# rpacheco-blazquez/PINN-FEM

Measured on AMD Instinct MI355X. Metric: element-residual-grad evals/sec (PINN+GD iteration: MLP fwd+bwd, stiffness, assembly, residual, Adam), collinear truss, higher is better.
Workload: dtype f32; 1 GPU; ex4 shape (nets (20, 15, 10), E and A evaluated), 1000000 elements per GPU, collinear 2-D truss h=1, alpha_data=100 with measurements at every node, load factor 0.1; elements_total=1000000, parallelism=elements sharded x1

## Files before the change

### include/pinnfem_hip.h

```cpp
#ifndef PINNFEM_HIP_H
#define PINNFEM_HIP_H

#include <stdint.h>

#ifdef __cplusplus
extern "C" {
#endif

#define PF_ABI_VERSION 8

#define PF_OK 0
#define PF_ERR_ARG (-1)
#define PF_ERR_UNSUPPORTED (-2)
#define PF_ERR_HIP (-3)

#define PF_DOF_FIXED 1u
#define PF_DOF_MEASURED 2u
#define PF_DOF_SHARED 4u
#define PF_DOF_GHOST 8u

#define PF_WG_SHUFFLE 0
#define PF_WG_MFMA 1
#define PF_WG_MFMA44 2
#define PF_WG_MFMA32 3
// ... 61 lines not shown
  int32_t wg_mode;
  float lam;
  float alpha_physics, alpha_data;
  float lr_u, lr_t;
  double tol;
  double beta1, beta2, eps;
  int32_t use_data;
  int32_t max_iter;
  float* theta_pad;
  float* prop_e;
  float* prop_a;
  float* g_f;
  float* g_ea;
  float* grad_u;
  float* grad_theta;
  float* partials;
  float* hist;
  pf_state* state;
  int32_t n_part_blocks;
  int32_t pad_total;
  const int32_t* pad_index;
  float n_meas_f;
  int32_t fe_mode;
  const int32_t* shared_dofs;
  const int32_t* shared_slot;
  int32_t n_shared;
  int32_t n_iface;
  int32_t own_lo, own_hi;
  int32_t part_half;
  int32_t prop_double;
  float* net_op;
  int32_t op_off[2];
  int32_t coord_exp;
  int32_t mlp_dtype;
  float* elem_k;
  float* theta_alt;
  float* u_alt;
  const int32_t* adj_other;
} pf_problem;

#define PF_MAX_BLOCKS 1024
#define PF_MAX_NODE_BLOCKS 4096
#define PF_NODE_SLOTS (PF_MAX_NODE_BLOCKS + 8)

int pf_abi_version(void);
const char* pf_last_error(void);
int pf_net_param_count(int in_dim, int width, int n_hidden);
int pf_padded_width(int width);
int pf_net_pad_count(int in_dim, int width, int n_hidden);
int pf_net_pad_index(int in_dim, int width, int n_hidden, int local);
int pf_sizeof(int what);
int pf_net_op_count(int in_dim, int width, int n_hidden);
long long pf_partials_count(const pf_problem* p);
#define PF_FUSED_FORWARD 1
#define PF_FUSED_BACKWARD 2
#define PF_FUSED_THETA_UPDATE 4
#define PF_FUSED_U_PINGPONG 8
#define PF_FUSED_U_UPDATE 16
int pf_fusion_info(const pf_problem* p);

int pf_pack_theta(const pf_problem* p, void* stream);
int pf_net_forward(const pf_problem* p, int which, void* stream);
int pf_net_forward_all(const pf_problem* p, void* stream);
int pf_net_backward_all(const pf_problem* p, void* stream);
int pf_internal_force(const pf_problem* p, const float* u, float* f_int_out, void* stream);
int pf_node_residual(const pf_problem* p, float* f_int_out, void* stream);
int pf_elem_adjoint(const pf_problem* p, void* stream);
int pf_net_backward(const pf_problem* p, int which, void* stream);
int pf_node_gradu(const pf_problem* p, int fuse_adam, void* stream);
int pf_theta_reduce(const pf_problem* p, int fuse_adam, void* stream);
int pf_finalize(const pf_problem* p, void* stream);
int pf_reset(const pf_problem* p, void* stream);

int pf_gd_iterations(const pf_problem* p, int n_iter, void* stream);
int pf_graph_create(const pf_problem* p, int iters_per_graph, void* stream, void** graph_out);
#define PF_GRAPH_CONT_HEAD 1
#define PF_GRAPH_NO_TAIL 2
int pf_graph_create_ex(const pf_problem* p, int iters_per_graph, int flags, void* stream, void** graph_out);
int pf_graph_tail(const pf_problem* p, int iters_per_graph, void* stream);
int pf_graph_launch(void* graph, void* stream);
int pf_graph_destroy(void* graph);
#define PF_KERNEL_SLOTS 9
int pf_gd_iterations_timed(const pf_problem* p, int n_iter, void* stream, float* ms_per_kernel);
int pf_loss_and_grads(const pf_problem* p, void* stream);

int pf_shard_forward(const pf_problem* p, void* stream);
int pf_shard_backward(const pf_problem* p, float* buf, const float* u2_local, void* stream);
int pf_shard_update_interior(const pf_problem* p, void* stream);
int pf_shard_update_shared(const pf_problem* p, const float* buf, float* u2_local, void* stream);
int pf_shard_flush(const pf_problem* p, const float* u2_reduced, void* stream);

#define PF_COMM_ID_BYTES 128
int pf_comm_unique_id(const char* librccl_path, void* id_out);
int pf_comm_create(const char* librccl_path, const void* id, int rank, int world, void** comm_out);
int pf_comm_destroy(void* comm);
int pf_comm_abort(void* comm);
int pf_comm_info(void* comm, int* rank_out, int* nranks_out);
int pf_comm_all_reduce(void* comm, float* buf, int n, void* stream);
int pf_shard_iterations(const pf_problem* p, void* comm, int n_iter, float* buf, float* u2_local, void* stream);
int pf_shard_graph_create(const pf_problem* p, void* comm, int iters_per_graph, float* buf, float* u2_local, void* stream,
                          void** graph_out);
int pf_shard_iterations_graph(const pf_problem* p, void* comm, void* graph, int iters_per_graph, int n_iter, float* buf,
                              float* u2_local, void* stream);

int pf_kv_f64(const pf_problem* p, const double* v, double* out, int zero_fixed, void* stream);
long long pf_pcg_workspace_count(const pf_problem* p);
// ... 53 lines not shown
```

### pinn_fem_amd/_capi.py

```python
from __future__ import annotations

import ctypes as C
import os

_HERE = os.path.dirname(os.path.abspath(__file__))
LIB_PATH = os.environ.get("PINNFEM_LIB") or os.path.join(_HERE, "lib", "libpinnfem_hip.so")

PF_ABI_VERSION = 8
PF_OK, PF_ERR_ARG, PF_ERR_UNSUPPORTED, PF_ERR_HIP = 0, -1, -2, -3
PF_DOF_FIXED, PF_DOF_MEASURED, PF_DOF_SHARED, PF_DOF_GHOST = 1, 2, 4, 8
PF_WG_SHUFFLE, PF_WG_MFMA, PF_WG_MFMA44, PF_WG_MFMA32 = 0, 1, 2, 3
PF_N32_WIDTH_MAX = 30
PF_MLP_F32, PF_MLP_BF16 = 0, 1
PF_FE_REFERENCE, PF_FE_DELTA = 0, 1
PF_HIST_COLS = 6
PF_MAX_BLOCKS = 1024
PF_COMM_ID_BYTES = 128
PF_MAX_NODE_BLOCKS = 4096
PF_NODE_SLOTS = PF_MAX_NODE_BLOCKS + 8
PF_KERNEL_SLOTS = 9
PF_COARSE_MAX_AGG, PF_COARSE_MODES = 256, 3
PF_COARSE_MAX = PF_COARSE_MAX_AGG * PF_COARSE_MODES
PF_GRAPH_CONT_HEAD, PF_GRAPH_NO_TAIL = 1, 2
PF_FUSED_FORWARD, PF_FUSED_BACKWARD, PF_FUSED_THETA_UPDATE, PF_FUSED_U_PINGPONG, PF_FUSED_U_UPDATE = 1, 2, 4, 8, 16
# ... 40 lines not shown
        ("theta", C.c_void_p), ("m_t", C.c_void_p), ("v_t", C.c_void_p),
        ("n_theta", C.c_int32), ("n_theta_active", C.c_int32),
        ("tensor_off", C.c_void_p),
        ("n_tensors", C.c_int32), ("wg_mode", C.c_int32),
        ("lam", C.c_float), ("alpha_physics", C.c_float), ("alpha_data", C.c_float),
        ("lr_u", C.c_float), ("lr_t", C.c_float),
        ("tol", C.c_double), ("beta1", C.c_double), ("beta2", C.c_double), ("eps", C.c_double),
        ("use_data", C.c_int32), ("max_iter", C.c_int32),
        ("theta_pad", C.c_void_p), ("prop_e", C.c_void_p), ("prop_a", C.c_void_p),
        ("g_f", C.c_void_p), ("g_ea", C.c_void_p), ("grad_u", C.c_void_p),
        ("grad_theta", C.c_void_p), ("partials", C.c_void_p), ("hist", C.c_void_p),
        ("state", C.c_void_p),
        ("n_part_blocks", C.c_int32), ("pad_total", C.c_int32),
        ("pad_index", C.c_void_p),
        ("n_meas_f", C.c_float), ("fe_mode", C.c_int32),
        ("shared_dofs", C.c_void_p), ("shared_slot", C.c_void_p),
        ("n_shared", C.c_int32), ("n_iface", C.c_int32),
        ("own_lo", C.c_int32), ("own_hi", C.c_int32), ("part_half", C.c_int32), ("prop_double", C.c_int32),
        ("net_op", C.c_void_p), ("op_off", C.c_int32 * 2), ("coord_exp", C.c_int32), ("mlp_dtype", C.c_int32),
        ("elem_k", C.c_void_p), ("theta_alt", C.c_void_p), ("u_alt", C.c_void_p), ("adj_other", C.c_void_p),
    ]


class PfScalarId(C.Structure):
    _fields_ = [
        ("p", C.c_void_p), ("m_p", C.c_void_p), ("v_p", C.c_void_p), ("table", C.c_void_p),
        ("n_rows", C.c_int32), ("has_bounds", C.c_int32),
        ("lo", C.c_float * 2), ("hi", C.c_float * 2),
        ("inv_ea0", C.c_float), ("lr_p", C.c_float), ("n_free_f", C.c_float), ("_pad", C.c_float),
    ]


class PfCoarse(C.Structure):
    _fields_ = [
        ("n_agg", C.c_int32), ("n_coarse", C.c_int32),
        ("node_agg", C.c_void_p), ("agg_off", C.c_void_p), ("zcoef", C.c_void_p),
        ("agg_ptr", C.c_void_p), ("agg_nodes", C.c_void_p), ("a_inv", C.c_void_p),
    ]


_PP = C.POINTER(PfProblem)
_PC = C.POINTER(PfCoarse)
SYMBOLS = {
    "pf_abi_version": (C.c_int, []),
    "pf_last_error": (C.c_char_p, []),
    "pf_net_param_count": (C.c_int, [C.c_int, C.c_int, C.c_int]),
    "pf_padded_width": (C.c_int, [C.c_int]),
    "pf_net_pad_count": (C.c_int, [C.c_int, C.c_int, C.c_int]),
    "pf_net_pad_index": (C.c_int, [C.c_int, C.c_int, C.c_int, C.c_int]),
    "pf_sizeof": (C.c_int, [C.c_int]),
    "pf_net_op_count": (C.c_int, [C.c_int, C.c_int, C.c_int]),
    "pf_partials_count": (C.c_longlong, [_PP]),
    "pf_fusion_info": (C.c_int, [_PP]),
    "pf_pack_theta": (C.c_int, [_PP, C.c_void_p]),
    "pf_net_forward": (C.c_int, [_PP, C.c_int, C.c_void_p]),
    "pf_net_forward_all": (C.c_int, [_PP, C.c_void_p]),
    "pf_net_backward_all": (C.c_int, [_PP, C.c_void_p]),
    "pf_internal_force": (C.c_int, [_PP, C.c_void_p, C.c_void_p, C.c_void_p]),
    "pf_node_residual": (C.c_int, [_PP, C.c_void_p, C.c_void_p]),
    "pf_elem_adjoint": (C.c_int, [_PP, C.c_void_p]),
    "pf_net_backward": (C.c_int, [_PP, C.c_int, C.c_void_p]),
    "pf_node_gradu": (C.c_int, [_PP, C.c_int, C.c_void_p]),
    "pf_theta_reduce": (C.c_int, [_PP, C.c_int, C.c_void_p]),
    "pf_finalize": (C.c_int, [_PP, C.c_void_p]),
    "pf_reset": (C.c_int, [_PP, C.c_void_p]),
    "pf_gd_iterations": (C.c_int, [_PP, C.c_int, C.c_void_p]),
    "pf_graph_create": (C.c_int, [_PP, C.c_int, C.c_void_p, C.POINTER(C.c_void_p)]),
    "pf_graph_create_ex": (C.c_int, [_PP, C.c_int, C.c_int, C.c_void_p, C.POINTER(C.c_void_p)]),
    "pf_graph_tail": (C.c_int, [_PP, C.c_int, C.c_void_p]),
    "pf_graph_launch": (C.c_int, [C.c_void_p, C.c_void_p]),
    "pf_graph_destroy": (C.c_int, [C.c_void_p]),
    "pf_gd_iterations_timed": (C.c_int, [_PP, C.c_int, C.c_void_p, C.POINTER(C.c_float)]),
    "pf_loss_and_grads": (C.c_int, [_PP, C.c_void_p]),
    "pf_shard_forward": (C.c_int, [_PP, C.c_void_p]),
    "pf_shard_backward": (C.c_int, [_PP, C.c_void_p, C.c_void_p, C.c_void_p]),
    "pf_shard_flush": (C.c_int, [_PP, C.c_void_p, C.c_void_p]),
    "pf_shard_update_interior": (C.c_int, [_PP, C.c_void_p]),
    "pf_shard_update_shared": (C.c_int, [_PP, C.c_void_p, C.c_void_p, C.c_void_p]),
    "pf_kv_f64": (C.c_int, [_PP, C.c_void_p, C.c_void_p, C.c_int, C.c_void_p]),
    "pf_pcg_workspace_count": (C.c_longlong, [_PP]),
    "pf_pcg_begin": (C.c_int, [_PP, C.c_void_p, C.c_void_p, C.c_void_p, C.c_double, C.c_void_p]),
    "pf_pcg_iterations": (C.c_int, [_PP, C.c_void_p, C.c_void_p, C.c_int, C.POINTER(C.c_double), C.c_void_p]),
    "pf_pcg_graph_create": (C.c_int, [_PP, C.c_void_p, C.c_void_p, C.c_int, C.c_void_p, C.POINTER(C.c_void_p)]),
    "pf_pcg_state": (C.c_int, [_PP, C.c_void_p, C.POINTER(C.c_double), C.c_void_p]),
    "pf_coarse_setup": (C.c_int, [_PP, _PC, C.c_void_p, C.c_void_p]),
    "pf_pcg2_workspace_count": (C.c_longlong, [_PP]),
    "pf_pcg2_begin": (C.c_int, [_PP, _PC, C.c_void_p, C.c_void_p, C.c_void_p, C.c_double, C.c_void_p]),
    "pf_pcg2_iterations": (C.c_int, [_PP, _PC, C.c_void_p, C.c_void_p, C.c_int, C.POINTER(C.c_double), C.c_void_p]),
    "pf_pcg2_graph_create": (C.c_int, [_PP, _PC, C.c_void_p, C.c_void_p, C.c_int, C.c_void_p, C.POINTER(C.c_void_p)]),
    "pf_pcg2_state": (C.c_int, [_PP, C.c_void_p, C.POINTER(C.c_double), C.c_void_p]),
    "pf_comm_unique_id": (C.c_int, [C.c_char_p, C.c_void_p]),
    "pf_comm_create": (C.c_int, [C.c_char_p, C.c_void_p, C.c_int, C.c_int, C.POINTER(C.c_void_p)]),
    "pf_comm_destroy": (C.c_int, [C.c_void_p]),
    "pf_comm_abort": (C.c_int, [C.c_void_p]),
    "pf_comm_info": (C.c_int, [C.c_void_p, C.POINTER(C.c_int), C.POINTER(C.c_int)]),
    "pf_comm_all_reduce": (C.c_int, [C.c_void_p, C.c_void_p, C.c_int, C.c_void_p]),
    "pf_shard_iterations": (C.c_int, [_PP, C.c_void_p, C.c_int, C.c_void_p, C.c_void_p, C.c_void_p]),
    "pf_shard_graph_create": (C.c_int, [_PP, C.c_void_p, C.c_int, C.c_void_p, C.c_void_p, C.c_void_p,
                                        C.POINTER(C.c_void_p)]),
    "pf_shard_iterations_graph": (C.c_int, [_PP, C.c_void_p, C.c_void_p, C.c_int, C.c_int, C.c_void_p, C.c_void_p,
                                            C.c_void_p]),
    "pf_scalar_gd_iterations": (C.c_int, [_PP, C.POINTER(PfScalarId), C.c_int, C.c_void_p]),
    "pf_adam": (C.c_int, [C.c_void_p, C.c_void_p, C.c_void_p, C.c_void_p, C.c_int, C.c_int,
                          C.c_double, C.c_double, C.c_double, C.c_double, C.c_void_p]),
    "pf_diag_k": (C.c_int, [_PP, C.c_void_p, C.c_void_p]),
    "pf_dense_k": (C.c_int, [_PP, C.c_void_p, C.c_void_p]),
# ... 54 lines not shown
```

### pinn_fem_amd/csrc/pf_api.hip

```cpp
#include <stdlib.h>
#include <string.h>
#include <stdio.h>
#include "pf_common.h"
#include "pf_net32.h"

int pf_launch_node_residual(const pf_problem* p, float* f_int_out, int compute_loss, hipStream_t s, int fin_prev = 0);
int pf_launch_elem_adjoint(const pf_problem* p, hipStream_t s);
int pf_launch_node_gradu(const pf_problem* p, int fuse_adam, hipStream_t s, int skip_shared = 0, float* u_out = nullptr);
int pf_launch_u_home(const pf_problem* p, hipStream_t s);
int pf_launch_scalar_residual(const pf_problem* p, const pf_scalar_id* sp, hipStream_t s);
int pf_launch_scalar_update(const pf_problem* p, const pf_scalar_id* sp, hipStream_t s);
int pf_launch_shard_pack(const pf_problem* p, float* buf2, const float* u2_local, hipStream_t s);
int pf_launch_shard_update(const pf_problem* p, const float* buf2, float* u2_local, hipStream_t s);
int pf_launch_shard_flush(const pf_problem* p, const float* u2, hipStream_t s);
int pf_launch_theta_reduce(const pf_problem* p, int fuse_adam, hipStream_t s);
int pf_launch_pack_theta(const pf_problem* p, hipStream_t s);
int pf_launch_finalize(const pf_problem* p, int mode, int with_theta, hipStream_t s, int tn_ready = 0);
int pf_launch_theta_stage1(const pf_problem* p, hipStream_t s);
int pf_launch_theta_stage2(const pf_problem* p, int fuse_adam, hipStream_t s);
int pf_launch_reset(const pf_problem* p, hipStream_t s);
int pf_launch_adam(float* param, const float* grad, float* m, float* v, int n, int step, double lr,
                   double beta1, double beta2, double eps, hipStream_t s);
int pf_launch_diag_k(const pf_problem* p, float* diag, hipStream_t s);
int pf_launch_dense_k(const pf_problem* p, float* K, hipStream_t s);
// ... 213 lines not shown
int pf_abi_version(void) { return PF_ABI_VERSION; }
const char* pf_last_error(void) { return g_err; }

int pf_sizeof(int what) {
  switch (what) {
    case 0: return (int)sizeof(pf_mesh);
    case 1: return (int)sizeof(pf_net);
    case 2: return (int)sizeof(pf_state);
    case 3: return (int)sizeof(pf_problem);
    case 4: return (int)sizeof(pf_scalar_id);
    case 5: return (int)sizeof(pf_coarse);
  }
  return PF_ERR_ARG;
}

int pf_net_param_count(int in_dim, int width, int n_hidden) {
  if (in_dim < 1 || width < 1 || n_hidden < 1) return PF_ERR_ARG;
  return width * in_dim + width + (n_hidden - 1) * (width * width + width) + width + 1;
}

int pf_padded_width(int width) { return padded_width(width); }

int pf_net_pad_count(int in_dim, int width, int n_hidden) {
  const int hp = padded_width(width);
  if (hp < 0 || n_hidden < 1 || n_hidden > 3 || (in_dim != 2 && in_dim != 3)) return PF_ERR_UNSUPPORTED;
  return pf_pad_count(hp, n_hidden);
}

int pf_net_pad_index(int in_dim, int width, int n_hidden, int local) {
  const int hp = padded_width(width);
  if (hp < 0 || n_hidden < 1 || n_hidden > 3 || (in_dim != 2 && in_dim != 3)) return PF_ERR_UNSUPPORTED;
  int q = local;
  if (q < 0) return PF_ERR_ARG;
  if (q < width * in_dim) return (q / in_dim) * 4 + (q % in_dim);
  q -= width * in_dim;
  if (q < width) return q * 4 + in_dim;
  q -= width;
  for (int l = 2; l <= n_hidden; ++l) {
    if (q < width * width) return pf_pad_wh(hp, l) + (q / width) * (hp + 4) + (q % width);
    q -= width * width;
    if (q < width) return pf_pad_wh(hp, l) + q * (hp + 4) + hp;
    q -= width;
  }
  if (q < width) return pf_pad_wo(hp, n_hidden) + q;
  q -= width;
  if (q == 0) return pf_pad_wo(hp, n_hidden) + hp;
  return PF_ERR_ARG;
}

int pf_net_op_count(int in_dim, int width, int n_hidden) {
  if (width < 1 || width > PF_N32_WIDTH_MAX || n_hidden < 1 || n_hidden > 3 || (in_dim != 2 && in_dim != 3))
    return PF_ERR_UNSUPPORTED;
  return (pf_n32_bytes(n_hidden) + 3) / 4;
}

long long pf_partials_count(const pf_problem* p) {
  if (!p) return PF_ERR_ARG;
  return (long long)PF_PART_WG + ((long long)p->n_part_blocks + PF_RG) * (long long)p->pad_total;
}

int pf_fusion_info(const pf_problem* p) {
  if (check_problem(p) != PF_OK) return PF_ERR_ARG;
  int m = 0;
  if (can_fuse_forward(p)) m |= PF_FUSED_FORWARD;
  if (can_fuse_backward(p)) m |= PF_FUSED_BACKWARD;
  if (can_fuse_theta_update(p)) m |= PF_FUSED_THETA_UPDATE;
  if (p->prop_double != 0 && p->elem_k != nullptr && can_fuse_gradu(p)) m |= PF_FUSED_U_UPDATE;
  else if (p->u_alt != nullptr && p->mesh.n_elems >= PF_GRAPH_DAG_MIN_ELEMS) m |= PF_FUSED_U_PINGPONG;
  return m;
}

int pf_pack_theta(const pf_problem* p, void* stream) {
  int rc = check_problem(p);
  if (rc) return rc;
  PF_TRY(pf_launch_pack_theta(p, (hipStream_t)stream), "pf_pack_theta");
  return PF_OK;
}

int pf_net_forward(const pf_problem* p, int which, void* stream) {
  int rc = check_problem(p);
  if (rc) return rc;
  if (which < 0 || which > 1 || !p->net[which].enabled) return fail(PF_ERR_ARG, "net not enabled");
  PF_TRY(net_forward(p, which, (hipStream_t)stream), "pf_net_forward");
  return PF_OK;
}

int pf_net_forward_all(const pf_problem* p, void* stream) {
  int rc = check_problem(p);
  if (rc) return rc;
  PF_TRY(net_forward_all(p, (hipStream_t)stream), "pf_net_forward_all");
  return PF_OK;
}

int pf_net_backward_all(const pf_problem* p, void* stream) {
  int rc = check_problem(p);
  if (rc) return rc;
  if (!(p->net[0].enabled || p->net[1].enabled)) return PF_OK;
  return enqueue_backwards(p, (hipStream_t)stream);
}

int pf_internal_force(const pf_problem* p, const float* u, float* f_int_out, void* stream) {
  int rc = check_problem(p);
  if (rc) return rc;
  if (!u || !f_int_out) return fail(PF_ERR_ARG, "null u / f_int_out");
  pf_problem q = *p;
  q.u = const_cast<float*>(u);
// ... 502 lines not shown
```

### pinn_fem_amd/csrc/pf_net32.h

```cpp
#pragma once
#include "pf_common.h"

#define PF_N32_MAX_WIDTH 30
#define PF_N32_KA 2048.0f
#define PF_N32_KW 16.0f
#define PF_N32_KB 16.0f
__host__ __device__ inline float pf_n32_lam_scale(float lam) {
  const float a = lam < 0.f ? -lam : lam;
  if (!(a > 0.f) || !(a < 3.0e38f)) return 1.0f;
  int ex = 0;
  (void)frexpf(a, &ex);
  ex = ex < -100 ? -100 : ex;
  return ldexpf(1.0f, 14 - ex);
}

__host__ __device__ constexpr int pf_n32_off_w1() { return 16; }
__host__ __device__ constexpr int pf_n32_off_wo() { return 16 + 512; }
__host__ __device__ constexpr int pf_n32_off_bo() { return 16 + 512 + 128; }
__host__ __device__ constexpr int pf_n32_off_layers() { return 16 + 512 + 128 + 16; }
#define PF_N32_LAYER_BYTES (128 + 4096 + 4096)
__host__ __device__ constexpr int pf_n32_off_bias(int l) { return pf_n32_off_layers() + (l - 2) * PF_N32_LAYER_BYTES; }
__host__ __device__ constexpr int pf_n32_off_af(int l) { return pf_n32_off_bias(l) + 128; }
__host__ __device__ constexpr int pf_n32_off_ab(int l) { return pf_n32_off_af(l) + 4096; }
__host__ __device__ constexpr int pf_n32_bytes(int n_hidden) { return pf_n32_off_layers() + (n_hidden - 1) * PF_N32_LAYER_BYTES; }
// ... 37 lines not shown
      unsigned short hf[8], hb[8];
#pragma unroll
      for (int j = 0; j < 8; ++j) {
        const int u_k = 2 * (8 * ks + j) + hh;
        float vf = 0.f, vb = 0.f;
        if (u_row < W && u_k < W) {
          vf = PF_N32_KW * Wl[u_row * W + u_k];
          vb = PF_N32_KB * Wl[u_k * W + u_row];
        }
        if (prec == 1) {
          hf[j] = sp ? (unsigned short)0 : __builtin_bit_cast(unsigned short, (__bf16)vf);
          hb[j] = sp ? (unsigned short)0 : __builtin_bit_cast(unsigned short, (__bf16)vb);
        } else {
          const _Float16 fh = (_Float16)vf, bh = (_Float16)vb;
          hf[j] = __builtin_bit_cast(unsigned short, sp ? (_Float16)(vf - (float)fh) : fh);
          hb[j] = __builtin_bit_cast(unsigned short, sp ? (_Float16)(vb - (float)bh) : bh);
        }
      }
      af[i] = make_uint4(hf[0] | (unsigned)hf[1] << 16, hf[2] | (unsigned)hf[3] << 16, hf[4] | (unsigned)hf[5] << 16,
                         hf[6] | (unsigned)hf[7] << 16);
      ab[i] = make_uint4(hb[0] | (unsigned)hb[1] << 16, hb[2] | (unsigned)hb[3] << 16, hb[4] | (unsigned)hb[5] << 16,
                         hb[6] | (unsigned)hb[7] << 16);
    }
  }
  if (with_bound && (tid >> 6) == ((nt - 1) >> 6)) {
    const int lane = tid & 63;
    float v = lane < W ? fabsf(th[o_wo + lane]) : 0.f;
    float bound = 0.f, grow = 1.f;
    for (int l = L; l >= 1; --l) {
      float m = v;
#pragma unroll
      for (int d = 32; d >= 1; d >>= 1) m = fmaxf(m, __shfl_xor(m, d));
      bound = fmaxf(bound, grow * m);
      grow *= 4.f;
      if (l >= 2) {
        const float* Wl = th + o_h + (l - 2) * per;
        float a = 0.f;
#pragma unroll 4
        for (int j = 0; j < W; ++j) {
          const float w = lane < W ? fabsf(Wl[j * W + lane]) : 0.f;
          a += w * __shfl(v, j);
        }
        v = a;
      }
    }
    if (lane == 0) {
      float* hdr = reinterpret_cast<float*>(img);
      hdr[0] = bound > 0.f ? bound : 1.f;
      hdr[1] = hdr[2] = hdr[3] = 0.f;
    }
  }
}

#define PF_FWD32_MAX_BLOCKS 256
inline int pf_n32_fwd2_blocks(int n_elems) {
  int nb = (n_elems + 1023) / 1024;
  if (nb > PF_FWD32_MAX_BLOCKS) nb = PF_FWD32_MAX_BLOCKS;
  if (nb < 1) nb = 1;
  return nb;
}
#define PF_GU_M 2
inline bool pf_n32_fwd2_can_update_u(const pf_problem* p, int gu_nb) {
  if (!p->adj_other || !p->m_u || !p->v_u || p->mesh.n_elems <= 0) return false;
  if (p->n_shared != 0 || p->own_lo != 0 || p->own_hi != 0) return false;
  const int nb = pf_n32_fwd2_blocks(p->mesh.n_elems);
  if (nb > gu_nb) return false;
  const int ntasks = (p->mesh.n_nodes + 64 * PF_GU_M - 1) / (64 * PF_GU_M);
  return (ntasks + nb - 1) / nb <= 1024 - 16;
}
```

### pinn_fem_amd/csrc/pf_net32.hip

```cpp
#include <type_traits>
#include <stdlib.h>
#include "pf_net32.h"
#include "pf_node.h"

#ifndef PF_NR
#error "compile with -DPF_NR=<registers per lane>"
#endif
#ifndef PF_PREC
#define PF_PREC 0
#endif
#ifndef PF_N32_DBG_ENABLE
#define PF_N32_DBG_ENABLE 0
#endif
#define PF_CAT2(a, b) a##b
#define PF_CAT(a, b) PF_CAT2(a, b)

typedef _Float16 h2 __attribute__((ext_vector_type(2)));
typedef _Float16 h8 __attribute__((ext_vector_type(8)));
typedef short s4v __attribute__((ext_vector_type(4)));
typedef float f32x16 __attribute__((ext_vector_type(16)));
typedef unsigned u32x4 __attribute__((ext_vector_type(4)));
typedef unsigned u32x2 __attribute__((ext_vector_type(2)));
typedef __bf16 bf2 __attribute__((ext_vector_type(2)));
typedef __bf16 bf8 __attribute__((ext_vector_type(8)));
// ... 905 lines not shown
  const float v = pf_wave_sum(gbo);
  if (lane == 0) mine[L * 1024 + 32] = v;
}
template <int NR, int L, int IN>
__device__ __forceinline__ void bw_row_from_parked(const pf_problem& P, int which, int hp, const float* __restrict__ park,
                                                   float kl, float kx) {
  const pf_net net = P.net[which];
  const int waves = blockDim.x >> 6, W = net.width;
  constexpr int PS = bw_park_floats<L>();
  float* __restrict__ prow = P.partials + PF_PART_WG + (size_t)blockIdx.x * P.pad_total + net.pad_off;
  const int padc = pf_pad_count(hp, L);
  for (int i = threadIdx.x; i < padc; i += blockDim.x) prow[i] = 0.f;
  __syncthreads();
  sfor<0, L>([&](auto l) {
    constexpr int LL = l + 1;
    float sc = 1.f;
    for (int k = 0; k < L - LL; ++k) sc *= 4.f;
    for (int idx = threadIdx.x; idx < 1024; idx += blockDim.x) {
      const int m = idx >> 5, c = idx & 31;
      const int j = 2 * (m & 15) + (m >> 4);
      if ((m & 15) >= NR || j >= W) continue;
      float t = 0.f;
      for (int q = 0; q < waves; ++q) t += park[q * PS + (LL - 1) * 1024 + idx];
      int dst = -1;
      float k = sc;
      if (LL >= 2) {
        const int kk = 2 * (c & 15) + (c >> 4);
        k *= PF_N32_KA;
        if (c == 15) dst = pf_pad_wh(hp, LL) + j * (hp + 4) + hp;
        else if ((c & 15) < NR && kk < W) dst = pf_pad_wh(hp, LL) + j * (hp + 4) + kk;
      } else {
        if (c < IN) { dst = j * 4 + c; k *= c == 0 ? kl : kx; }
        else if (c == IN) dst = j * 4 + IN;
      }
      if (dst >= 0) prow[dst] = t / k;
    }
  });
  float* const pwo = prow + pf_pad_wo(hp, L);
  if (threadIdx.x < 32) {
    const int hh = threadIdx.x >> 4, r = threadIdx.x & 15, u = 2 * r + hh;
    if (r < NR && u < W) {
      float t = 0.f;
      for (int q = 0; q < waves; ++q) t += park[q * PS + L * 1024 + hh * 16 + r];
      pwo[u] = t * (1.0f / PF_N32_KA);
    }
  }
  if (threadIdx.x == 32) {
    float t = 0.f;
    for (int q = 0; q < waves; ++q) t += park[q * PS + L * 1024 + 32];
    pwo[hp] = t;
  }
}

template <int NR, int L, int IN, bool GEA, int MODE = 0, class FirstRow = int>
__device__ __forceinline__ void backward_phase(const pf_problem& P, int which, int hp, int dbg, const unsigned char* smem,
                                               unsigned char* cst, unsigned char* wscr,
                                               unsigned long long* stamps = nullptr, float* park = nullptr,
                                               FirstRow first_row = FirstRow(), int shift8 = 0) {
  using E = Eng<NR>;
  constexpr int CONST_BYTES = E::CONST_BYTES, WAVE_SCRATCH = E::WAVE_SCRATCH, REGION = E::REGION, NPK = E::NPK;
  constexpr bool COMPACT = E::COMPACT;
  typedef typename E::WriteBase WriteBase;
  constexpr int DIM = IN - 1;
  const pf_net net = P.net[which];
  const pf_net onet = P.net[1 - which];
  const float* __restrict__ other = which == 0 ? P.prop_a : P.prop_e;
  const float* __restrict__ mine = which == 0 ? P.prop_e : P.prop_a;
  const int n = P.mesh.n_elems;
  const int lane = threadIdx.x & 63, wv = threadIdx.x >> 6, waves = blockDim.x >> 6;
  const int h = lane >> 5;
  unsigned char* scratch = wscr + wv * WAVE_SCRATCH;
  if constexpr (MODE != 2)
    for (int i = threadIdx.x; i < CONST_BYTES / 4; i += blockDim.x) reinterpret_cast<unsigned*>(cst)[i] = 0u;
  for (int i = lane; i < WAVE_SCRATCH / 16; i += 64) reinterpret_cast<uint4*>(scratch)[i] = make_uint4(0, 0, 0, 0);
  if constexpr (MODE != 2) __syncthreads();
  if (MODE != 2 && threadIdx.x < 32)
    if constexpr (COMPACT)
      *reinterpret_cast<unsigned short*>(cst + 192 + REGION + 64 * (threadIdx.x >> 2) + 8 * (threadIdx.x & 3) + 6) = BF ? 0x4500 : 0x6800;
  const unsigned char* rd = E::operand_base(scratch, lane, cst + 192);
  const WriteBase wb = E::write_base(scratch, lane);

  const int per_round = (int)gridDim.x * waves;
  const int ntasks_all = (n + 63) >> 6;
  const int slot = (int)blockIdx.x * waves + wv;
  const int hw = waves >> 1;
  const bool elder = wv < hw;
  const int partner = elder ? slot + hw : slot - hw;
  const int c_own = slot < ntasks_all ? (ntasks_all - 1 - slot) / per_round + 1 : 0;
  const int c_par = (hw > 0 && partner < ntasks_all) ? (ntasks_all - 1 - partner) / per_round + 1 : 0;
  const int sh = min((shift8 > 0 && hw > 0 && (waves & 1) == 0) ? (((elder ? c_par : c_own) * shift8 + 4) >> 3) : 0,
                     elder ? c_par : c_own);
  const int n_mine = elder ? c_own + sh : c_own - sh;
  auto task_base = [&](int k) {
    if (k < (elder ? c_own : n_mine)) return (k * per_round + slot) * 64;
    if (elder && k < n_mine) return ((c_par - sh + (k - c_own)) * per_round + partner) * 64;
    return n - 1;
  };
  TaskIn<DIM> nxt;
  int2 nn_ahead = int2{0, 0};
  if (n > 0) {
    task_fetch_a<IN, GEA>(nxt, P, onet, other, mine, min(task_base(0) + lane, n - 1));
    if (GEA) nn_ahead = reinterpret_cast<const int2*>(P.mesh.conn)[min(task_base(1) + lane, n - 1)];
  }
  if constexpr (MODE != 2) __syncthreads();
  task_fetch_b<IN, GEA>(nxt, P);

  const float bound = __builtin_bit_cast(float, __builtin_amdgcn_readfirstlane(__builtin_bit_cast(int, reinterpret_cast<const float*>(smem)[0])));
  const float kx = __builtin_bit_cast(float, __builtin_amdgcn_readfirstlane(__builtin_bit_cast(int, __builtin_ldexpf(1.0f, P.coord_exp))));
  const float inv_scale = __builtin_bit_cast(float, __builtin_amdgcn_readfirstlane(__builtin_bit_cast(int, 1.0f / net.scale)));
  const float kl = __builtin_bit_cast(float, __builtin_amdgcn_readfirstlane(__builtin_bit_cast(int, pf_n32_lam_scale(P.lam))));
  f32x16 T[L];
  sfor<0, L>([&](auto l) { constexpr int LL = l; T[LL] = zero16(); });
  float Srun = 0.f;
  float go[NR];
  sfor<0, NR>([&](auto r) { constexpr int R = r; go[R] = 0.f; });
  float gbo = 0.f;

  if (PF_N32_DBG_ENABLE && stamps) stamps[0] = __builtin_amdgcn_s_memrealtime();
  for (int k = 0; k < n_mine; ++k) {
    const int base = task_base(k);
    const int e = base + lane;
    const bool live = e < n;
    const TaskIn<DIM> cur = nxt;
    const bool more = k + 1 < n_mine;
    float gz = 0.f;
    if (live) {
      float gea;
      if (GEA) {
        gea = task_gea<DIM>(cur, P.fe_mode);
        P.g_ea[e] = gea;
      } else {
        gea = cur.gea;
      }
      float g = gea * cur.oth;
      g = g * net.scale;
      gz = net.positive ? g * one_minus_exp_neg(cur.own * inv_scale) : g;
    }
    const float gabs = fabsf(gz) * bound;
    if (Srun == 0.f || __builtin_amdgcn_ballot_w64(gabs * Srun >= 16384.0f) != 0ull) {
      const float gmax = wave_max(gabs);
      if (gmax > 0.f && gmax < 3.0e38f) {
        int ex = 0;
        (void)frexpf(gmax, &ex);
        ex = ex < -100 ? -100 : (ex > 100 ? 100 : ex);
        const float Sneed = __builtin_ldexpf(1.0f, 14 - ex);
        if (Srun == 0.f) Srun = Sneed;
        else if (Sneed < Srun) {
          const float f = Sneed / Srun;
          sfor<0, L>([&](auto l) {
            constexpr int LL = l;
            sfor<0, 16>([&](auto i) { constexpr int I = i; T[LL][I] *= f; });
          });
          Srun = Sneed;
        }
      }
    }
    const float S = Srun == 0.f ? 1.0f : Srun;
    float g0, g1;
    both_tiles(gz, g0, g1);
    float xa0, xa1, xb0, xb1;
    both_tiles(cur.x[1], xa0, xa1);
    both_tiles(cur.x[2], xb0, xb1);
    const float lam_in = cur.x[0];
    if (more) {
      task_fetch_a<IN, GEA>(nxt, P, onet, other, mine, min(task_base(k + 1) + lane, n - 1), false);
      if (GEA) {
        nxt.nn = nn_ahead;
        task_fetch_b<IN, GEA>(nxt, P);
        nn_ahead = reinterpret_cast<const int2*>(P.mesh.conn)[min(task_base(k + 2) + lane, n - 1)];
      }
    }
    auto tile_backward = [&](const typename E::template TileAct<L, true>& A, const float (&xt)[3], float gt, bool go_done) {
      unsigned xhi[NPK], xlo[NPK];
      sfor<2, NPK>([&](auto q) { constexpr int Q = q; xhi[Q] = 0u; xlo[Q] = 0u; });
      split_pair(kl * xt[0], kx * xt[1], xhi[0], xlo[0]);
      split_pair(IN == 3 ? kx * xt[2] : 1.0f, IN == 3 ? 1.0f : 0.f, xhi[1], xlo[1]);
      if (!go_done) sfor<0, NR>([&](auto r) { constexpr int R = r; go[R] = fmaf(gt, A.aL[R], go[R]); });
      if (!(dbg & 2)) E::template backward_tile<L, IN>(smem, scratch, lane, A, gt * S, xhi, xlo, T, wb, rd, dbg);
    };
    if constexpr (E::template bw_pair<L>()) {
      const float x0[3] = {lam_in, xa0, xb0}, x1[3] = {lam_in, xa1, xb1};
      typename E::template TileAct<L, true> A0, A1;
      float p0, p1;
      E::template forward_tiles<L, IN, true>(smem, lane, x0, x1, A0, A1, p0, p1, 0, -1, go, g0, g1);
      tile_backward(A0, x0, g0, true);
      tile_backward(A1, x1, g1, true);
    } else {
      sfor<0, 2>([&](auto tt) {
        constexpr int TT = tt;
        const float xt[3] = {lam_in, TT ? xa1 : xa0, TT ? xb1 : xb0};
        typename E::template TileAct<L, true> A;
        E::template recompute_tile<L, IN>(smem, lane, xt, A);
        tile_backward(A, xt, TT ? g1 : g0, false);
      });
    }
    gbo += gz;
  }
  if (PF_N32_DBG_ENABLE && stamps) stamps[1] = __builtin_amdgcn_s_memrealtime();
  const float invS = Srun == 0.f ? 1.0f : 1.0f / Srun;
  sfor<0, L>([&](auto l) {
    constexpr int LL = l;
    sfor<0, 16>([&](auto i) { constexpr int I = i; T[LL][I] *= invS; });
  });
  if constexpr (MODE == 1) {
    bw_park<NR, L>(park + (size_t)wv * bw_park_floats<L>(), T, go, gbo, lane);
    if (PF_N32_DBG_ENABLE && stamps) stamps[2] = __builtin_amdgcn_s_memrealtime();
    return;
  } else if constexpr (MODE == 2) {
    __syncthreads();
    first_row();
    __syncthreads();
    bw_park<NR, L>(park + (size_t)wv * bw_park_floats<L>(), T, go, gbo, lane);
    __syncthreads();
    bw_row_from_parked<NR, L, IN>(P, which, hp, park, kl, kx);
    if (PF_N32_DBG_ENABLE && stamps) stamps[2] = __builtin_amdgcn_s_memrealtime();
    return;
  }

  __syncthreads();
  float* stage = reinterpret_cast<float*>(wscr);
  const int W = net.width;
// ... 44 lines not shown
    if (lane == 0) stage[waves * 64 + wv] = v;
  }
  __syncthreads();
  float* const pwo = prow + pf_pad_wo(hp, L);
  if (threadIdx.x < 32) {
    const int hh = threadIdx.x >> 4, r = threadIdx.x & 15, u = 2 * r + hh;
    if (r < NR && u < W) {
      float t = 0.f;
      for (int q = 0; q < waves; ++q) t += stage[q * 64 + hh * 16 + r];
      pwo[u] = t * (1.0f / PF_N32_KA);
    }
  }
  if (threadIdx.x == 32) {
    float t = 0.f;
    for (int q = 0; q < waves; ++q) t += stage[waves * 64 + q];
    pwo[hp] = t;
  }
  if (PF_N32_DBG_ENABLE && stamps) stamps[2] = __builtin_amdgcn_s_memrealtime();
}


template <int NR, int L, int IN, bool GEA>
__global__ __launch_bounds__((Eng<NR>::template bw_threads<L, GEA>())) void k_net32_backward(pf_problem P, int which, int hp, int dbg_arg) {
  using E = Eng<NR>;
  const int dbg = PF_N32_DBG_ENABLE ? dbg_arg : 0;
  extern __shared__ __align__(16) unsigned char smem[];
  constexpr int IMG = pf_n32_bytes(L), IMGPAD = (IMG + 255) & ~255;
  __shared__ int s_done;
  if (threadIdx.x == 0) s_done = P.state->done;
  copy_image(smem, reinterpret_cast<const unsigned char*>(P.net_op + P.op_off[which]), IMG);
  __syncthreads();
  if (s_done != 0 || P.mesh.n_elems <= 0) return;
  backward_phase<NR, L, IN, GEA>(P, which, hp, dbg, smem, smem + IMGPAD, smem + IMGPAD + E::CONST_BYTES);
}

template <int NRE, int NRA, int L, int IN>
constexpr int bw2_threads() {
  return Eng<NRE>::template bw_threads<L, true>() < Eng<NRA>::template bw_threads<L, false>()
             ? Eng<NRE>::template bw_threads<L, true>() : Eng<NRA>::template bw_threads<L, false>();
}
template <int NRE, int NRA>
constexpr int bw2_const_bytes() { return Eng<NRE>::CONST_BYTES > Eng<NRA>::CONST_BYTES ? Eng<NRE>::CONST_BYTES : Eng<NRA>::CONST_BYTES; }
template <int NRE, int NRA>
constexpr int bw2_wave_scratch() { return Eng<NRE>::WAVE_SCRATCH > Eng<NRA>::WAVE_SCRATCH ? Eng<NRE>::WAVE_SCRATCH : Eng<NRA>::WAVE_SCRATCH; }

template <int NRE, int NRA>
constexpr bool bw2_parked() { return Eng<NRE>::COMPACT && Eng<NRA>::COMPACT; }
template <int NRE, int NRA, int L, int IN>
constexpr size_t bw2_lds_bytes() {
  return 2 * (size_t)((pf_n32_bytes(L) + 255) & ~255) + bw2_const_bytes<NRE, NRA>() +
         (size_t)(bw2_threads<NRE, NRA, L, IN>() / 64) * bw2_wave_scratch<NRE, NRA>() +
         (bw2_parked<NRE, NRA>() ? (size_t)(bw2_threads<NRE, NRA, L, IN>() / 64) * bw_park_floats<L>() * sizeof(float) : 0);
}
constexpr int PF_BW_SHIFT = 2;
template <int NRE, int NRA, int L, int IN>
__global__ __launch_bounds__((bw2_threads<NRE, NRA, L, IN>())) void k_net32_backward2(pf_problem P, int hp_e, int hp_a, int dbg_arg) {
  const int dbg = PF_N32_DBG_ENABLE ? dbg_arg : 0;
  const unsigned long long t_entry = PF_N32_DBG_ENABLE ? __builtin_amdgcn_s_memrealtime() : 0ull;
  extern __shared__ __align__(16) unsigned char smem[];
  constexpr int IMG = pf_n32_bytes(L), IMGPAD = (IMG + 255) & ~255;
  __shared__ int s_done;
  if (threadIdx.x == 0) s_done = P.state->done;
  copy_images2(smem, reinterpret_cast<const unsigned char*>(P.net_op + P.op_off[0]), smem + IMGPAD,
               reinterpret_cast<const unsigned char*>(P.net_op + P.op_off[1]), IMG);
  __syncthreads();
  if (s_done != 0 || P.mesh.n_elems <= 0) return;
  unsigned char* cst = smem + 2 * IMGPAD;
  unsigned char* wscr = cst + bw2_const_bytes<NRE, NRA>();
  unsigned long long* st = nullptr;
  if (PF_N32_DBG_ENABLE && (dbg & 16) && (threadIdx.x & 63) == 0) {
    st = reinterpret_cast<unsigned long long*>(P.u_alt) + 65536 + (size_t)(blockIdx.x * (blockDim.x >> 6) + (threadIdx.x >> 6)) * 8;
    st[0] = t_entry;
  }
  if constexpr (bw2_parked<NRE, NRA>()) {
    float* park = reinterpret_cast<float*>(wscr + (size_t)(blockDim.x >> 6) * bw2_wave_scratch<NRE, NRA>());
    const float kl_e = pf_n32_lam_scale(P.lam), kx_e = __builtin_ldexpf(1.0f, P.coord_exp);
    auto first_row = [&]() { bw_row_from_parked<NRE, L, IN>(P, 0, hp_e, park, kl_e, kx_e); };
    backward_phase<NRE, L, IN, true, 1>(P, 0, hp_e, dbg, smem, cst, wscr, st ? st + 1 : nullptr, park, 0, PF_BW_SHIFT);
    backward_phase<NRA, L, IN, false, 2>(P, 1, hp_a, dbg, smem + IMGPAD, cst, wscr, st ? st + 4 : nullptr, park, first_row,
                                         PF_BW_SHIFT);
  } else {
    backward_phase<NRE, L, IN, true>(P, 0, hp_e, dbg, smem, cst, wscr, st ? st + 1 : nullptr, nullptr, 0, PF_BW_SHIFT);
    __syncthreads();
    backward_phase<NRA, L, IN, false>(P, 1, hp_a, dbg, smem + IMGPAD, cst, wscr, st ? st + 4 : nullptr, nullptr, 0, PF_BW_SHIFT);
  }
}

template <int L, int IN>
int launch_fwd(const pf_problem* p, int which, hipStream_t s, int s2_half) {
  constexpr int NR = PF_NR;
  const int nb = pf_n32_fwd2_blocks(p->mesh.n_elems);
  static const int dbg = getenv("PF_N32_DBG") ? atoi(getenv("PF_N32_DBG")) : 0;
  const int ws = p->elem_k != nullptr ? 1 : 0;
  const size_t lds = s2_half < 0 ? (size_t)pf_n32_bytes(L)
                                 : (size_t)((pf_n32_bytes(L) + 255) & ~255) + (size_t)p->n_theta_active * sizeof(float);
  if (lds > 64000) { pf_set_error("too many trainable parameters for the fused theta update"); return PF_ERR_UNSUPPORTED; }
  hipLaunchKernelGGL((k_net32_forward<NR, L, IN>), dim3(nb), dim3(FW_THREADS), lds, s, *p, which, dbg, ws, s2_half);
  return hipGetLastError() == hipSuccess ? PF_OK : PF_ERR_HIP;
}

template <int L, int IN, bool GEA>
int launch_bwd_t(const pf_problem* p, int which, hipStream_t s) {
  const int nb = pf_net_blocks(p);
  const int hp = ((p->net[which].width + 3) / 4) * 4;
  constexpr int NR = PF_NR;
  using E = Eng<NR>;
  constexpr int BW_THREADS = E::template bw_threads<L, GEA>();
  const size_t lds = ((pf_n32_bytes(L) + 255) & ~255) + E::CONST_BYTES + (size_t)(BW_THREADS / 64) * E::WAVE_SCRATCH;
  static_assert(E::WAVE_SCRATCH >= 4096 + 512, "write-out staging must fit the wave scratch");
  static const int dbg = getenv("PF_N32_DBG") ? atoi(getenv("PF_N32_DBG")) : 0;
  hipLaunchKernelGGL((k_net32_backward<NR, L, IN, GEA>), dim3(nb), dim3(BW_THREADS), lds, s, *p, which, hp, dbg);
  return hipGetLastError() == hipSuccess ? PF_OK : PF_ERR_HIP;
}
template <int L, int IN>
int launch_bwd(const pf_problem* p, int which, hipStream_t s) { return launch_bwd_t<L, IN, false>(p, which, s); }
template <int L, int IN>
int launch_bwd_gea(const pf_problem* p, int which, hipStream_t s) { return launch_bwd_t<L, IN, true>(p, which, s); }

template <int NRA, int L, int IN>
int launch_fwd2_t(const pf_problem* p, hipStream_t s, const pf_fwd2_opts& o) {
  const int s2_half = o.s2_half, gu_nb = o.gu_nb;
  constexpr int NRE = PF_NR;
  const int n = p->mesh.n_elems;
  const int nb = pf_n32_fwd2_blocks(n);
  static const int dbg = getenv("PF_N32_DBG") ? atoi(getenv("PF_N32_DBG")) : 0;
  const size_t lds = 2 * (size_t)((pf_n32_bytes(L) + 255) & ~255) + (s2_half < 0 ? 0 : (size_t)p->n_theta_active * sizeof(float));
  if (lds > 64000) { pf_set_error("too many trainable parameters for the fused theta update"); return PF_ERR_UNSUPPORTED; }
  if (gu_nb > 0 && !pf_n32_fwd2_can_update_u(p, gu_nb)) { pf_set_error("fused forward: displacement update not possible on this problem"); return PF_ERR_UNSUPPORTED; }
  hipLaunchKernelGGL((k_net32_forward2<NRE, NRA, L, IN>), dim3(nb), dim3(FW_THREADS), lds, s, *p, dbg, s2_half >= 0 && o.calc_index ? s2_half + 2 : s2_half, gu_nb, o.gu_k);
  return hipGetLastError() == hipSuccess ? PF_OK : PF_ERR_HIP;
}
template <int L, int IN>
int launch_fwd2(const pf_problem* p, hipStream_t s, const pf_fwd2_opts& o) {
  switch (pf_net32_bucket(p->net[1].width)) {
    case 2: return launch_fwd2_t<2, L, IN>(p, s, o);
    case 4: return launch_fwd2_t<4, L, IN>(p, s, o);
    case 6: return launch_fwd2_t<6, L, IN>(p, s, o);
// ... 109 lines not shown
```

Measured before the change: 7.707 billion element-evals/s.

## Rebalance backward wave task assignment with dealt tails and refetched g_ea

Replaces the proportional shift-based work stealing between paired waves in the fused two-network backward kernel with a new walk scheme. Leftover tasks are dealt across waves, rotated between the E and A phases, and each pair shifts a fixed handicap of tasks. The A phase now recomputes g_ea from connectivity and displacements instead of reading the stored value, which changes the phase-to-phase dependency and the load pattern. A host helper is exported so the task assignment can be checked. The intent is to cut wave imbalance and tail idle time, at the cost of extra gathers and compute in the A phase.

```diff
diff --git a/include/pinnfem_hip.h b/include/pinnfem_hip.h
--- a/include/pinnfem_hip.h
+++ b/include/pinnfem_hip.h
@@ -137,6 +137,7 @@
 int pf_sizeof(int what);
 int pf_net_op_count(int in_dim, int width, int n_hidden);
 long long pf_partials_count(const pf_problem* p);
+long long pf_bw2_assignment(int n_elems, int blocks, int waves, int phase, int32_t* slot_out, int32_t* pos_out);
 #define PF_FUSED_FORWARD 1
 #define PF_FUSED_BACKWARD 2
 #define PF_FUSED_THETA_UPDATE 4
diff --git a/pinn_fem_amd/_capi.py b/pinn_fem_amd/_capi.py
--- a/pinn_fem_amd/_capi.py
+++ b/pinn_fem_amd/_capi.py
@@ -116,6 +116,7 @@
     "pf_net_op_count": (C.c_int, [C.c_int, C.c_int, C.c_int]),
     "pf_partials_count": (C.c_longlong, [_PP]),
     "pf_fusion_info": (C.c_int, [_PP]),
+    "pf_bw2_assignment": (C.c_longlong, [C.c_int, C.c_int, C.c_int, C.c_int, C.c_void_p, C.c_void_p]),
     "pf_pack_theta": (C.c_int, [_PP, C.c_void_p]),
     "pf_net_forward": (C.c_int, [_PP, C.c_int, C.c_void_p]),
     "pf_net_forward_all": (C.c_int, [_PP, C.c_void_p]),
diff --git a/pinn_fem_amd/csrc/pf_api.hip b/pinn_fem_amd/csrc/pf_api.hip
--- a/pinn_fem_amd/csrc/pf_api.hip
+++ b/pinn_fem_amd/csrc/pf_api.hip
@@ -289,6 +289,26 @@
   if (width < 1 || width > PF_N32_WIDTH_MAX || n_hidden < 1 || n_hidden > 3 || (in_dim != 2 && in_dim != 3))
     return PF_ERR_UNSUPPORTED;
   return (pf_n32_bytes(n_hidden) + 3) / 4;
+}
+
+long long pf_bw2_assignment(int n_elems, int blocks, int waves, int phase, int32_t* slot_out, int32_t* pos_out) {
+  if (n_elems < 0 || blocks < 1 || waves < 1 || (phase != 0 && phase != 1) || !slot_out || !pos_out)
+    return fail(PF_ERR_ARG, "pf_bw2_assignment: bad argument");
+  if ((long long)blocks * waves > (1 << 24)) return fail(PF_ERR_ARG, "pf_bw2_assignment: grid too large");
+  const int ntasks = (n_elems + 63) >> 6;
+  for (int t = 0; t < ntasks; ++t) slot_out[t] = pos_out[t] = -1;
+  long long walked = 0;
+  for (int b = 0; b < blocks; ++b)
+    for (int w = 0; w < waves; ++w) {
+      const pf_bw_walk wk = pf_bw_walk_of(n_elems, blocks, waves, b, w, phase);
+      for (int k = 0; k < wk.n_walk; ++k, ++walked) {
+        const int t = pf_bw_task(n_elems, blocks, waves, b, w, phase, k);
+        if (t < 0 || t >= ntasks) return fail(PF_ERR_ARG, "pf_bw2_assignment: task out of range");
+        slot_out[t] = b * waves + w;
+        pos_out[t] = k;
+      }
+    }
+  return walked;
 }
 
 long long pf_partials_count(const pf_problem* p) {
diff --git a/pinn_fem_amd/csrc/pf_net32.h b/pinn_fem_amd/csrc/pf_net32.h
--- a/pinn_fem_amd/csrc/pf_net32.h
+++ b/pinn_fem_amd/csrc/pf_net32.h
@@ -113,6 +113,73 @@
   }
 }
 
+#ifndef PF_BW_HANDICAP_E
+#define PF_BW_HANDICAP_E 2
+#endif
+#ifndef PF_BW_HANDICAP_A
+#define PF_BW_HANDICAP_A 2
+#endif
+#define PF_BW_PHASE_PLAIN (-1)
+
+struct pf_bw_walk {
+  int n_walk;
+  int n_own;
+  int par_first;
+  int rounds, per_round;
+  int slot, partner;
+  int own_tail, par_tail;
+};
+
+__host__ __device__ inline int pf_bw_deal_index(int grid, int waves, int block, int wave, int off) {
+  const int hw = waves >> 1, npairs = grid * hw;
+  const int second = wave >= hw ? 1 : 0;
+  int jj = (wave - second * hw) * grid + block - off;
+  if (jj < 0) jj += npairs;
+  return jj + second * npairs;
+}
+
+__host__ __device__ inline pf_bw_walk pf_bw_walk_of(int n_elems, int grid, int waves, int block, int wave, int phase) {
+  pf_bw_walk w;
+  const int per_round = grid * waves, ntasks = n_elems > 0 ? (n_elems + 63) >> 6 : 0;
+  const int hw = waves >> 1;
+  const bool paired = phase >= 0 && hw > 0 && (waves & 1) == 0;
+  const bool elder = wave < hw;
+  const int slot = block * waves + wave;
+  const int partner = !paired ? slot : (elder ? slot + hw : slot - hw);
+  const int rounds = ntasks / per_round, r = ntasks - rounds * per_round;
+  const bool dealt = paired && rounds >= 1;
+  const int off = (dealt && phase == 1) ? r % (grid * hw) : 0;
+  const int j_own = dealt ? pf_bw_deal_index(grid, waves, block, wave, off) : slot;
+  const int j_par = dealt ? pf_bw_deal_index(grid, waves, block, elder ? wave + hw : wave - hw, off) : partner;
+  w.rounds = rounds;
+  w.per_round = per_round;
+  w.slot = slot;
+  w.partner = partner;
+  w.own_tail = j_own < r ? rounds * per_round + j_own : -1;
+  w.par_tail = (paired && j_par < r) ? rounds * per_round + j_par : -1;
+  const int c_own = rounds + (j_own < r ? 1 : 0);
+  const int c_par = paired ? rounds + (j_par < r ? 1 : 0) : 0;
+  const int c_young = elder ? c_par : c_own;
+  const int handicap = phase == 0 ? PF_BW_HANDICAP_E : PF_BW_HANDICAP_A;
+  const int half = c_young >> 1;
+  const int sh = !paired ? 0 : (handicap < half ? handicap : half);
+  w.n_own = elder ? c_own : c_own - sh;
+  w.n_walk = elder ? c_own + sh : c_own - sh;
+  w.par_first = c_par - sh;
+  return w;
+}
+
+__host__ __device__ inline int pf_bw_walk_task(const pf_bw_walk& w, int k) {
+  if (k < 0 || k >= w.n_walk) return -1;
+  const bool own = k < w.n_own;
+  const int i = own ? k : w.par_first + (k - w.n_own);
+  return i < w.rounds ? i * w.per_round + (own ? w.slot : w.partner) : (own ? w.own_tail : w.par_tail);
+}
+
+__host__ __device__ inline int pf_bw_task(int n_elems, int grid, int waves, int block, int wave, int phase, int k) {
+  return pf_bw_walk_task(pf_bw_walk_of(n_elems, grid, waves, block, wave, phase), k);
+}
+
 #define PF_FWD32_MAX_BLOCKS 256
 inline int pf_n32_fwd2_blocks(int n_elems) {
   int nb = (n_elems + 1023) / 1024;
diff --git a/pinn_fem_amd/csrc/pf_net32.hip b/pinn_fem_amd/csrc/pf_net32.hip
--- a/pinn_fem_amd/csrc/pf_net32.hip
+++ b/pinn_fem_amd/csrc/pf_net32.hip
@@ -981,16 +981,17 @@
   }
 }
 
-template <int NR, int L, int IN, bool GEA, int MODE = 0, class FirstRow = int>
+template <int NR, int L, int IN, bool GEA, int MODE = 0, bool REGEA = false, class FirstRow = int>
 __device__ __forceinline__ void backward_phase(const pf_problem& P, int which, int hp, int dbg, const unsigned char* smem,
                                                unsigned char* cst, unsigned char* wscr,
                                                unsigned long long* stamps = nullptr, float* park = nullptr,
-                                               FirstRow first_row = FirstRow(), int shift8 = 0) {
+                                               FirstRow first_row = FirstRow(), int phase = PF_BW_PHASE_PLAIN) {
   using E = Eng<NR>;
   constexpr int CONST_BYTES = E::CONST_BYTES, WAVE_SCRATCH = E::WAVE_SCRATCH, REGION = E::REGION, NPK = E::NPK;
   constexpr bool COMPACT = E::COMPACT;
   typedef typename E::WriteBase WriteBase;
   constexpr int DIM = IN - 1;
+  constexpr bool FETCH = GEA || REGEA;
   const pf_net net = P.net[which];
   const pf_net onet = P.net[1 - which];
   const float* __restrict__ other = which == 0 ? P.prop_a : P.prop_e;
@@ -1009,30 +1010,29 @@
   const unsigned char* rd = E::operand_base(scratch, lane, cst + 192);
   const WriteBase wb = E::write_base(scratch, lane);
 
-  const int per_round = (int)gridDim.x * waves;
-  const int ntasks_all = (n + 63) >> 6;
-  const int slot = (int)blockIdx.x * waves + wv;
-  const int hw = waves >> 1;
-  const bool elder = wv < hw;
-  const int partner = elder ? slot + hw : slot - hw;
-  const int c_own = slot < ntasks_all ? (ntasks_all - 1 - slot) / per_round + 1 : 0;
-  const int c_par = (hw > 0 && partner < ntasks_all) ? (ntasks_all - 1 - partner) / per_round + 1 : 0;
-  const int sh = min((shift8 > 0 && hw > 0 && (waves & 1) == 0) ? (((elder ? c_par : c_own) * shift8 + 4) >> 3) : 0,
-                     elder ? c_par : c_own);
-  const int n_mine = elder ? c_own + sh : c_own - sh;
+  pf_bw_walk wk = pf_bw_walk_of(n, (int)gridDim.x, waves, (int)blockIdx.x, wv, phase);
+  wk.n_walk = __builtin_amdgcn_readfirstlane(wk.n_walk);
+  wk.n_own = __builtin_amdgcn_readfirstlane(wk.n_own);
+  wk.par_first = __builtin_amdgcn_readfirstlane(wk.par_first);
+  wk.rounds = __builtin_amdgcn_readfirstlane(wk.rounds);
+  wk.per_round = __builtin_amdgcn_readfirstlane(wk.per_round);
+  wk.slot = __builtin_amdgcn_readfirstlane(wk.slot);
+  wk.partner = __builtin_amdgcn_readfirstlane(wk.partner);
+  wk.own_tail = __builtin_amdgcn_readfirstlane(wk.own_tail);
+  wk.par_tail = __builtin_amdgcn_readfirstlane(wk.par_tail);
+  const int n_mine = wk.n_walk;
   auto task_base = [&](int k) {
-    if (k < (elder ? c_own : n_mine)) return (k * per_round + slot) * 64;
-    if (elder && k < n_mine) return ((c_par - sh + (k - c_own)) * per_round + partner) * 64;
-    return n - 1;
+    const int t = pf_bw_walk_task(wk, k);
+    return t < 0 ? n - 1 : t * 64;
   };
   TaskIn<DIM> nxt;
   int2 nn_ahead = int2{0, 0};
   if (n > 0) {
-    task_fetch_a<IN, GEA>(nxt, P, onet, other, mine, min(task_base(0) + lane, n - 1));
-    if (GEA) nn_ahead = reinterpret_cast<const int2*>(P.mesh.conn)[min(task_base(1) + lane, n - 1)];
+    task_fetch_a<IN, FETCH>(nxt, P, onet, other, mine, min(task_base(0) + lane, n - 1));
+    if (FETCH) nn_ahead = reinterpret_cast<const int2*>(P.mesh.conn)[min(task_base(1) + lane, n - 1)];
   }
   if constexpr (MODE != 2) __syncthreads();
-  task_fetch_b<IN, GEA>(nxt, P);
+  task_fetch_b<IN, FETCH>(nxt, P);
 
   const float bound = __builtin_bit_cast(float, __builtin_amdgcn_readfirstlane(__builtin_bit_cast(int, reinterpret_cast<const float*>(smem)[0])));
   const float kx = __builtin_bit_cast(float, __builtin_amdgcn_readfirstlane(__builtin_bit_cast(int, __builtin_ldexpf(1.0f, P.coord_exp))));
@@ -1055,9 +1055,9 @@
     float gz = 0.f;
     if (live) {
       float gea;
-      if (GEA) {
+      if (FETCH) {
         gea = task_gea<DIM>(cur, P.fe_mode);
-        P.g_ea[e] = gea;
+        if (GEA) P.g_ea[e] = gea;
       } else {
         gea = cur.gea;
       }
@@ -1092,10 +1092,10 @@
     both_tiles(cur.x[2], xb0, xb1);
     const float lam_in = cur.x[0];
     if (more) {
-      task_fetch_a<IN, GEA>(nxt, P, onet, other, mine, min(task_base(k + 1) + lane, n - 1), false);
-      if (GEA) {
+      task_fetch_a<IN, FETCH>(nxt, P, onet, other, mine, min(task_base(k + 1) + lane, n - 1), false);
+      if (FETCH) {
         nxt.nn = nn_ahead;
-        task_fetch_b<IN, GEA>(nxt, P);
+        task_fetch_b<IN, FETCH>(nxt, P);
         nn_ahead = reinterpret_cast<const int2*>(P.mesh.conn)[min(task_base(k + 2) + lane, n - 1)];
       }
     }
@@ -1246,7 +1246,6 @@
          (size_t)(bw2_threads<NRE, NRA, L, IN>() / 64) * bw2_wave_scratch<NRE, NRA>() +
          (bw2_parked<NRE, NRA>() ? (size_t)(bw2_threads<NRE, NRA, L, IN>() / 64) * bw_park_floats<L>() * sizeof(float) : 0);
 }
-constexpr int PF_BW_SHIFT = 2;
 template <int NRE, int NRA, int L, int IN>
 __global__ __launch_bounds__((bw2_threads<NRE, NRA, L, IN>())) void k_net32_backward2(pf_problem P, int hp_e, int hp_a, int dbg_arg) {
   const int dbg = PF_N32_DBG_ENABLE ? dbg_arg : 0;
@@ -1270,13 +1269,14 @@
     float* park = reinterpret_cast<float*>(wscr + (size_t)(blockDim.x >> 6) * bw2_wave_scratch<NRE, NRA>());
     const float kl_e = pf_n32_lam_scale(P.lam), kx_e = __builtin_ldexpf(1.0f, P.coord_exp);
     auto first_row = [&]() { bw_row_from_parked<NRE, L, IN>(P, 0, hp_e, park, kl_e, kx_e); };
-    backward_phase<NRE, L, IN, true, 1>(P, 0, hp_e, dbg, smem, cst, wscr, st ? st + 1 : nullptr, park, 0, PF_BW_SHIFT);
-    backward_phase<NRA, L, IN, false, 2>(P, 1, hp_a, dbg, smem + IMGPAD, cst, wscr, st ? st + 4 : nullptr, park, first_row,
-                                         PF_BW_SHIFT);
+    backward_phase<NRE, L, IN, true, 1>(P, 0, hp_e, dbg, smem, cst, wscr, st ? st + 1 : nullptr, park, 0, 0);
+    backward_phase<NRA, L, IN, false, 2, true>(P, 1, hp_a, dbg, smem + IMGPAD, cst, wscr, st ? st + 4 : nullptr, park,
+                                               first_row, 1);
   } else {
-    backward_phase<NRE, L, IN, true>(P, 0, hp_e, dbg, smem, cst, wscr, st ? st + 1 : nullptr, nullptr, 0, PF_BW_SHIFT);
+    backward_phase<NRE, L, IN, true>(P, 0, hp_e, dbg, smem, cst, wscr, st ? st + 1 : nullptr, nullptr, 0, 0);
     __syncthreads();
-    backward_phase<NRA, L, IN, false>(P, 1, hp_a, dbg, smem + IMGPAD, cst, wscr, st ? st + 4 : nullptr, nullptr, 0, PF_BW_SHIFT);
+    backward_phase<NRA, L, IN, false, 0, true>(P, 1, hp_a, dbg, smem + IMGPAD, cst, wscr, st ? st + 4 : nullptr, nullptr,
+                                               0, 1);
   }
 }
 
```

Measured after the change: 7.520 billion element-evals/s. 0.976x the previous value.
